# spirit-man/Planetary-LiDAR-Odometry

Hardware: AMD Instinct MI355X
Metric: IMLS-ICP scan-pairs/s (HDL-64 ~120k-pt scan vs 10-scan map, 20 ICP iterations) (higher is better)
Workload: dtype f64; 1 GPU; config B: HDL-64 scan vs 10-scan local map; a step = 4 independent scan pairs as 4 launch sequences in flight; queries=126189, map_points=1262664, solver=LS (trimmed, t=0.02), search_number=20, inputs=resident in HBM, fused_launch=True, launch_groups=4, parallelism=1 GPU, no process group

## Files before the change

planetary-lidar-odometry_amd/csrc/internal.h:

```cpp
#pragma once
#include <cstddef>
#include <hip/hip_runtime.h>
#include <cstdint>
#include <string>
#include <vector>

#include "../../include/imls_gpu.h"

namespace imlsgpu {

constexpr int kBlock = 256;
constexpr int kProjBlock = 128;
constexpr int kStackDepth = 24;
constexpr int kHistBins = 65536;
constexpr int kCandCap = 8192;
constexpr int kNormEq = 28;

static_assert(sizeof(imls_iter_trace) == 16 * 8 * 2 + 8 * 8, "trace layout");

struct DevBuf {
    void* p = nullptr;
    size_t bytes = 0;
};

// ... 16 lines not shown
    double delta_dist, delta_angle;
    int matcher;
    int proj;
    double gate_dist, gate_proj;
    int qwave;
    int packet;
    int pk_small, pk_iters;
    int pk_batch;
    int reuse;
    int force_fb;
    int xcd;
    int tv;
    int tv_k;
    double tv_sigma, tv_thr;
    float tv_skin;
    int bfs;
};
#ifndef IMLS_BFS_ITERS
#define IMLS_BFS_ITERS 0
#endif
inline KParams kp_at(const KParams& k, int it) {
    KParams r = k;
    r.packet = it >= 0 && it < k.pk_iters ? k.pk_small : 64;
    r.bfs = it >= 0 && it < IMLS_BFS_ITERS;
    return r;
}
constexpr int kTvMaxK = 64;
constexpr int kTvList = 64;
constexpr size_t kTvBytesPerQuery = 32 + 16 + 4 * kTvList + 72;

struct TreeView {
    const float4* mpt;
    const float4* mnr;
    const unsigned* ipos;
    const float4* nodes;
    const float4* tpt;
    const float4* tnr;
    int M, B, P, levels;
    const unsigned long long* lkeys;
// ... 211 lines not shown
int fifo_merge(hipStream_t s, const unsigned long long* a, const unsigned* av, int na, const unsigned long long* b,
               unsigned bid, int nb, unsigned long long* okey, unsigned* oval, DevBuf& scratch, std::string& err);
int fifo_index(hipStream_t s, const unsigned long long* mkey, const unsigned* mval, int M, const FifoRunTable& runs,
               const float* fq, const unsigned* clamp, unsigned* h_clamp, int B, DevBuf& lkeys, DevBuf& mpt, DevBuf& nodes,
               DevBuf& treescratch, int* P_out, int* levels_out, std::string& err);

void launch_project(hipStream_t s, const TreeView& t, const float4* spt, const float4* snr,
                    const unsigned* qperm, int N, const double* pose, const int* done, const KParams& kp,
                    float4* cs, float4* cd, float4* cn, double* partial1, imls_iter_trace* tr,
                    unsigned long long* nbr_stats, unsigned* fb_list, unsigned* fb_count, int lane_mode,
                    const double* delta, int* lists, int use_prev, hipEvent_t* marks = nullptr);
constexpr int kMaxKL = 46;
__host__ __device__ inline float4* xref_of(int* lists, int N) {
    return reinterpret_cast<float4*>(reinterpret_cast<char*>(lists) + ((size_t)(kMaxKL + 1) * N * 4 + 255) / 256 * 256);
}
__host__ __device__ inline unsigned* cmp_of(int* lists, int N) {
    return reinterpret_cast<unsigned*>(reinterpret_cast<char*>(xref_of(lists, N)) + ((size_t)N * 20 + 255) / 256 * 256);
}
__host__ __device__ inline unsigned* cmp_count_of(int* lists, int N) { return cmp_of(lists, N) + ((size_t)N + 63) / 64 * 64; }
inline size_t prevnn_bytes(int N) {
    return ((size_t)(kMaxKL + 1) * N * 4 + 255) / 256 * 256 + ((size_t)N * 20 + 255) / 256 * 256 + ((size_t)N + 63) / 64 * 256 +
           ((size_t)N / 64 + 2) * 4 + 512;
}
constexpr int kStatSkipped = 6;
int project_blocks(int N);
#ifndef IMLS_FINISH_QUAD
#define IMLS_FINISH_QUAD 0
#endif
constexpr int kPass1Block = IMLS_FINISH_QUAD ? 64 : 256;
constexpr int kPass1Fallback = 64;
void launch_project_batch(hipStream_t s, const PairDev* tab, const int* n_host, int npairs, const KParams& kp, int it,
                          int use_prev);

void launch_solve_chain(hipStream_t s, int N, int blocks1, const KParams& kp, const float4* cs,
                        const float4* cd, const float4* cn, const double* rows_d, const double* weights,
                        SolveState& st, imls_iter_trace* tr, int update_pose, int rows_are_double,
                        const int* count = nullptr, const double* wsum = nullptr);
// ... 63 lines not shown
```

planetary-lidar-odometry_amd/csrc/project.hip:

```cpp
#include <algorithm>
#include <cfloat>

#include "internal.h"
#include "geom.h"

namespace imlsgpu {
namespace {

constexpr double kInfD = __builtin_huge_val();
constexpr float kInfF = __builtin_huge_valf();
constexpr int kWaveBlock = 256;
typedef float kf4v __attribute__((ext_vector_type(4)));
typedef __attribute__((address_space(4))) const kf4v kconst_f4;
__device__ __forceinline__ int ld_const(const int* p) { return *(const __attribute__((address_space(4))) int*)p; }
__device__ __forceinline__ double ld_const(const double* p) { return *(const __attribute__((address_space(4))) double*)p; }
constexpr int kFallbackBlocks = 64;
constexpr int kFallbackBlocksBatched = 4;
constexpr int kFinishPerBlock = IMLS_FINISH_QUAD ? kWaveBlock / 4 : kWaveBlock;
static_assert(kFinishPerBlock == kPass1Block && kFallbackBlocks == kPass1Fallback, "pass-1 slab layout (solve.hip)");
#ifndef IMLS_COMPACT
#define IMLS_COMPACT 0
#endif
constexpr int kWideMax = 8;
constexpr int kWaveStack = 64;
constexpr int kFStack = 256;
constexpr int kFBatchMax = 128;
static_assert(kFBatchMax + 64 + 7 * ((24 + 2) / 3) <= kFStack, "frontier stack bound");
#ifndef IMLS_SEED_CHUNK
#define IMLS_SEED_CHUNK 8
#endif
constexpr int kSeedChunk = IMLS_SEED_CHUNK;
constexpr int kSeedTab = 1024;
constexpr int kSeedHalf = 1;
constexpr float kReseed = 0.25f;
#ifndef IMLS_LEAF_PREFETCH
#define IMLS_LEAF_PREFETCH 1
#endif
// ... 336 lines not shown
#pragma unroll
    for (int j = 0; j < KL; ++j) {
        const float up = I::hi(lk[j]);
        const bool in = I::real(lk[j]) && up <= r2f;
        cnt_r += in ? 1 : 0;
        if (in && d1 == kInfF && I::lo(lk[j]) > 1e-15f) d1 = up;
        if (j == K - 1) dK = up;
    }
    return cnt_r >= K ? fmaxf(dK, d1) : (IMLS_UNDER_SKIN > 0 ? r2f : kInfF);
}

#ifndef IMLS_KNN_WAVES
#define IMLS_KNN_WAVES 5
#endif
#define IMLS_KNN_ATTR __attribute__((amdgpu_waves_per_eu(KL <= 26 ? IMLS_KNN_WAVES : 2)))
template <int KL, int MODE = 0>
__device__ __forceinline__ void knn_wave_body(TreeView t, const float4* __restrict__ spt,
                                                         const unsigned* __restrict__ qperm, int N,
                                                         const double* __restrict__ pose,
                                                         const int* __restrict__ done, KParams kp,
                                                         const double* __restrict__ delta,
                                                         int* __restrict__ lists, float* __restrict__ wlist,
                                                         float4* __restrict__ xref, float* __restrict__ nref,
                                                         int use_prev, unsigned long long* __restrict__ nbr_stats,
                                                         int bx, unsigned* __restrict__ cmp = nullptr,
                                                         unsigned* __restrict__ cmp_count = nullptr) {
    if (done && ld_const(done)) return;
    __shared__ int snode[kWaveBlock / 64][kWaveStack];
    __shared__ float4 sboxa[kWaveBlock / 64][kWaveStack];
    __shared__ float2 sboxb[kWaveBlock / 64][kWaveStack];
    __shared__ int spos[KL][kWaveBlock];
    const int tid = threadIdx.x, lane = tid & 63;
    int* const mypos = &spos[0][tid];
    using IK = IdKeys<KL>;
    const int wv = __builtin_amdgcn_readfirstlane(tid >> 6);
    const int qp = kp.packet;
    const int pslot = (bx * (kWaveBlock / 64) + wv) * qp + lane;
    int slot = pslot;
    bool active = lane < qp && slot < N;
    if constexpr (MODE == 2) {
        const int cnt = ld_const((const int*)cmp_count + bx);
        if (wv * qp >= cnt) return;
        active = lane < qp && wv * qp + lane < cnt;
        slot = active ? (int)cmp[(size_t)bx * (kWaveBlock / 64) * qp + wv * qp + lane] : 0;
    }
    float xf[3] = {0.f, 0.f, 0.f};
    float w_prev = 0.f, n_prev = 0.f;
    float4 x_prev = make_float4(0.f, 0.f, 0.f, 0.f);
    if (active) {
        double ns[3];
        const int i = (int)qperm[slot];
        const float4 sp4 = spt[i];
        if (use_prev) {
            w_prev = wlist[slot];
            x_prev = xref[slot];
            n_prev = nref[slot];
        }
        transform_query(pose, sp4, make_float4(0.f, 0.f, 0.f, 0.f), 0, xf, ns);
    }
    float lk[KL];
// ... 2 lines not shown
    if (use_prev) {
#pragma unroll
        for (int j = 0; j < KL; ++j) mypos[j * kWaveBlock] = -1;
    }
    auto thr_ = [&]() -> float { return IK::lo(lk[KL - 1]); };
    auto full_ = [&]() -> bool { return IK::real(lk[KL - 1]); };
    auto pos_ = [&](int s) -> int { return mypos[s * kWaveBlock]; };
    auto need_ = [&]() -> float { return need_key_ids<KL>(lk, (float)kp.r2, kp.K); };
    auto ins_ = [&](float d, int pos) {
        const unsigned s = IK::id(lk[KL - 1]);
        insert_key<KL>(lk, IK::make(d, s));
        mypos[s * kWaveBlock] = pos;
    };
    const float r2s = (float)(kp.r2 * kSearchR2) * kBoxSlack + 1e-30f;
    float bnd = active ? r2s : -1.0f;
    const int P = t.P, B = t.B, M = t.M;
#ifdef IMLS_DEBUG_WAVE_TRACE
    const long long dbg_t0 = wall_clock64();
#endif
    bool greedy = active && !use_prev;
    bool skip = false;
    float wskip = kInfF;
    if (active && use_prev) {
        double rf = 0.0;
#pragma unroll
        for (int r = 0; r < 3; ++r)
#pragma unroll
            for (int c = 0; c < 3; ++c) {
                const double e = ld_const(delta + r * 4 + c) - (r == c ? 1.0 : 0.0);
                rf += e * e;
            }
// ... 38 lines not shown
                for (int j = par; j + 1 < KL; j += 2) {
                    const bool sw = lk[j + 1] < lk[j];
                    const float tk = lk[j];
                    lk[j] = sw ? lk[j + 1] : lk[j];
                    lk[j + 1] = sw ? tk : lk[j + 1];
                    swapped |= sw;
                }
            }
        }
        bnd = fmin_nn(r2s, thr_());
        if (kp.reuse && wlow > 0.f) {
            const float nk = need_();
            if (nk < kInfF && nk * (1.0f + 1e-5f) < wlow) { skip = true; wskip = wlow; }
        }
    }
    if constexpr (MODE == 1) {
        if (active && skip) wlist[slot] = wskip;
        const unsigned long long sk = __ballot(skip);
        if (nbr_stats && lane == 0 && sk) atomicAdd(&nbr_stats[kStatSkipped], (unsigned long long)__popcll(sk));
        const bool need = active && !skip;
        const unsigned long long nm = __ballot(need);
        __shared__ int wneed[kWaveBlock / 64];
        if (lane == 0) wneed[wv] = __popcll(nm);
        __syncthreads();
        int off = 0, tot = 0;
#pragma unroll
        for (int w = 0; w < kWaveBlock / 64; ++w) {
            off += w < wv ? wneed[w] : 0;
            tot += wneed[w];
        }
        if (need) cmp[(size_t)bx * (kWaveBlock / 64) * qp + off + __popcll(nm & ((1ull << lane) - 1ull))] = (unsigned)slot;
        if (tid == 0) cmp_count[bx] = (unsigned)tot;
        return;
    }
#ifdef IMLS_DEBUG_WAVE_TRACE
    unsigned dbg_ev = 0, dbg_ins = 0;
    unsigned dbg_sparse = 0, dbg_bcast = 0, dbg_sparse_lanes = 0, dbg_sparse_ins = 0;
    unsigned dbg_seed_steps = 0, dbg_seed_pts = 0;
#endif
    auto scan_leaf = [&](int leaf, unsigned long long want, bool listed, float4 mine) {
        const int base = leaf * B;
        const int cnt = min(B, M - base);
        unsigned long long inl = 0ull;
        auto listed_mask = [&]() {
#pragma unroll
            for (int k = 0; k < KL; ++k) {
                const unsigned rel = (unsigned)(pos_(k) - base);
                inl |= rel < 64u ? (1ull << rel) : 0ull;
            }
        };
        const bool sparse = __popcll(want) <= kSparseLanes;
#ifdef IMLS_DEBUG_WAVE_TRACE
        if (sparse) { ++dbg_sparse; dbg_sparse_lanes += __popcll(want); } else { ++dbg_bcast; }
#endif
        if (sparse) {
            int nin = 0;
            bool have_inl = !listed;
            if (listed) {
#pragma unroll
                for (int k = 0; k < KL; ++k) nin += (unsigned)(pos_(k) - base) < (unsigned)cnt ? 1 : 0;
            }
            const float cb = fmin_nn(r2s, IK::hi(lk[KL - 1]));
            unsigned long long cm = 0ull;
            unsigned long long m = want;
            while (m) {
                const int q = __builtin_amdgcn_readfirstlane(__builtin_ctzll(m));
                m &= m - 1;
                const float qx = __int_as_float(__builtin_amdgcn_readlane(__float_as_int(xf[0]), q));
                const float qy = __int_as_float(__builtin_amdgcn_readlane(__float_as_int(xf[1]), q));
                const float qz = __int_as_float(__builtin_amdgcn_readlane(__float_as_int(xf[2]), q));
                const float qb = __int_as_float(__builtin_amdgcn_readlane(__float_as_int(cb), q));
                const float ex = mine.x - qx, ey = mine.y - qy, ez = mine.z - qz;
                const float d32 = __builtin_fmaf(ex, ex, __builtin_fmaf(ey, ey, ez * ez));
                unsigned long long pm = __ballot(lane < cnt && d32 <= qb);
                if (!have_inl) {
                    const int nq = __builtin_amdgcn_readlane(nin, q);
                    if (__popcll(pm) > nq) {
                        listed_mask();
                        have_inl = true;
                    } else {
                        pm = 0ull;
                    }
                }
                if (pm) {
                    const unsigned long long inq =
                        ((unsigned long long)(unsigned)__builtin_amdgcn_readlane((int)(unsigned)(inl >> 32), q) << 32) |
                        (unsigned)__builtin_amdgcn_readlane((int)(unsigned)inl, q);
                    pm &= ~inq;
                }
                if (lane == q) cm = pm;
            }
            while (__ballot(cm != 0ull)) {
                const int jj = cm ? (int)__builtin_ctzll(cm) : 0;
                const float px = __shfl(mine.x, jj), py = __shfl(mine.y, jj), pz = __shfl(mine.z, jj);
                if (cm) {
                    cm &= cm - 1;
                    const float ex = px - xf[0], ey = py - xf[1], ez = pz - xf[2];
                    const float d32 = __builtin_fmaf(ex, ex, __builtin_fmaf(ey, ey, ez * ez));
                    if (d32 <= bnd && d32 < thr_()) {
#ifdef IMLS_DEBUG_WAVE_TRACE
                        ++dbg_ins;
#endif
                        ins_(d32, base + jj);
                        bnd = fmin_nn(r2s, thr_());
                    }
                }
#ifdef IMLS_DEBUG_WAVE_TRACE
                ++dbg_ev;
#endif
            }
        } else {
            if (listed) listed_mask();
            const bool wants = (want >> lane) & 1ull;
#if IMLS_BCAST_SCALAR
            const kconst_f4* lp = (const kconst_f4*)t.mpt + base;
            kf4v g[kBcGroup];
#pragma unroll
            for (int u = 0; u < kBcGroup; ++u) g[u] = lp[min(u, cnt - 1)];
            for (int j0 = 0; j0 < cnt; j0 += kBcGroup) {
                kf4v nx[kBcGroup];
                const int jn = j0 + kBcGroup;
                if (jn + kBcGroup <= cnt) {
                    const kconst_f4* q = lp + jn;
#pragma unroll
                    for (int u = 0; u < kBcGroup; ++u) nx[u] = q[u];
                } else {
// ... 103 lines not shown
        }
    }
    unsigned n_inner = 0, n_leaf = 0;
#ifdef IMLS_DEBUG_WAVE_TRACE
    const long long dbg_t1 = wall_clock64();
#endif
    if (skip) bnd = -1.0f;
    int node = 1, sp = 0;
#if IMLS_LEAF_PREFETCH
    int pf_leaf = -1;
    float4 pf = make_float4(0.f, 0.f, 0.f, 0.f);
#endif
    unsigned long long em = __ballot(active && !skip);
    const unsigned long long skipped = __ballot(skip);
    if (nbr_stats && lane == 0 && skipped) atomicAdd(&nbr_stats[kStatSkipped], (unsigned long long)__popcll(skipped));
    if constexpr (MODE == 3) {
        if (em) {
            const bool walk = active && !skip;
            const float rr = walk ? sqrtf(bnd * kBoxSlack) * (1.0f + 1e-5f) + 1e-5f : 0.f;
            float plo[3], phi[3];
#pragma unroll
            for (int a = 0; a < 3; ++a) {
                plo[a] = walk ? xf[a] - rr : kInfF;
                phi[a] = walk ? xf[a] + rr : -kInfF;
            }
#pragma unroll
            for (int o = 1; o < 64; o <<= 1)
#pragma unroll
                for (int a = 0; a < 3; ++a) {
                    plo[a] = fminf(plo[a], __shfl_xor(plo[a], o, 64));
                    phi[a] = fmaxf(phi[a], __shfl_xor(phi[a], o, 64));
                }
            int fc = 1, lev = 0;
            if (lane == 0) snode[wv][0] = 1;
            while (lev < t.levels) {
                const int sw = min(kWide, t.levels - lev), nk = 1 << sw;
                const int below = t.levels - lev - sw;
                const int reserve = (kWideMax - 1) * ((below + kWide - 1) / kWide);
                const int n = lane < fc ? snode[wv][lane] : 0;
                const float4* rec = t.nodes + 3 * ((size_t)(n > 0 ? n : 1) << (sw - 1));
                auto child_box = [&](int k, float (&lo)[3], float (&hi)[3]) {
                    const float4 ra = rec[3 * (k >> 1)], rb = rec[3 * (k >> 1) + 1], rc = rec[3 * (k >> 1) + 2];
                    if (k & 1) { lo[0] = rb.z; lo[1] = rb.w; lo[2] = rc.x; hi[0] = rc.y; hi[1] = rc.z; hi[2] = rc.w; }
                    else { lo[0] = ra.x; lo[1] = ra.y; lo[2] = ra.z; hi[0] = ra.w; hi[1] = rb.x; hi[2] = rb.y; }
                };
                unsigned cm = 0u;
                if (lane < fc) {
#pragma unroll
                    for (int k = 0; k < kWideMax; ++k) {
                        if (k >= nk) break;
                        float lo[3], hi[3];
                        child_box(k, lo, hi);
                        const bool ov = lo[0] <= phi[0] && hi[0] >= plo[0] && lo[1] <= phi[1] && hi[1] >= plo[1] &&
                                        lo[2] <= phi[2] && hi[2] >= plo[2];
                        cm |= ov ? (1u << k) : 0u;
                    }
                }
                const int cnt = __popc(cm);
                int inc = cnt;
#pragma unroll
                for (int o = 1; o < 64; o <<= 1) {
                    const int v = __shfl_up(inc, o, 64);
                    if (lane >= o) inc += v;
                }
                const int total = __shfl(inc, 63, 64);
                if (total == 0 || total + reserve > kWaveStack) break;
                int off = inc - cnt;
                if (cm) {
#pragma unroll
                    for (int k = 0; k < kWideMax; ++k) {
                        if (!((cm >> k) & 1u)) continue;
                        float lo[3], hi[3];
                        child_box(k, lo, hi);
                        snode[wv][off] = (n << sw) + k;
                        sboxa[wv][off] = make_float4(lo[0], lo[1], lo[2], hi[0]);
                        sboxb[wv][off] = make_float2(hi[1], hi[2]);
                        ++off;
                    }
                }
                fc = total;
                lev += sw;
                ++n_inner;
            }
            if (lev > 0) {
                int en = 0;
                float4 ea = make_float4(0.f, 0.f, 0.f, 0.f);
                float2 eb = make_float2(0.f, 0.f);
                if (lane < fc) { en = snode[wv][lane]; ea = sboxa[wv][lane]; eb = sboxb[wv][lane]; }
                if (lane < fc) { snode[wv][fc - 1 - lane] = en; sboxa[wv][fc - 1 - lane] = ea; sboxb[wv][fc - 1 - lane] = eb; }
                sp = fc;
                node = 0;
                while (sp > 0) {
                    --sp;
                    const float4 b0 = sboxa[wv][sp];
                    const float2 b1 = sboxb[wv][sp];
                    const float d = box_d2(xf, b0.x, b0.y, b0.z, b0.w, b1.x, b1.y);
                    em = __ballot(d <= bnd * kBoxSlack);
                    if (em) { node = snode[wv][sp]; break; }
                }
                if (!node) em = 0ull;
            }
        }
    }
    while (em) {
        if (node < P) {
            ++n_inner;
            const int lev = 31 - __builtin_clz(node);
            const int sw = min(kWide, t.levels - lev);
            const int nk = 1 << sw, nrec = nk >> 1;
            const int unode = __builtin_amdgcn_readfirstlane(node);
            const kconst_f4* rec = (const kconst_f4*)t.nodes + 3 * ((size_t)unode << (sw - 1));
            float4 R[3 * (kWideMax / 2)];
#pragma unroll
            for (int k = 0; k < 3 * (kWideMax / 2); ++k) {
                const kf4v v = rec[min(k, 3 * nrec - 1)];
                R[k] = make_float4(v.x, v.y, v.z, v.w);
            }
            const float bs = bnd * kBoxSlack;
            unsigned long long m[kWideMax];
            int best = -1;
            float bd = kInfF;
#pragma unroll
            for (int k = 0; k < kWideMax; ++k) {
                const float4 a = R[3 * (k >> 1)], b = R[3 * (k >> 1) + 1], c = R[3 * (k >> 1) + 2];
                const float d = (k & 1) ? box_d2(xf, b.z, b.w, c.x, c.y, c.z, c.w) : box_d2(xf, a.x, a.y, a.z, a.w, b.x, b.y);
                const bool w = k < nk && d <= bs;
                m[k] = __ballot(w);
                if (w && d < bd) { bd = d; best = k; }
            }
            int cstar = -1, vbest = 0;
#pragma unroll
            for (int k = 0; k < kWideMax; ++k) {
                const int v = __popcll(__ballot(best == k));
                if (m[k] && (cstar < 0 || v > vbest)) { cstar = k; vbest = v; }
            }
            if (cstar >= 0) {
#pragma unroll
                for (int k = kWideMax - 1; k >= 0; --k) {
                    if (m[k] && k != cstar) {
                        if (lane == 0) {
                            const float4 a = R[3 * (k >> 1)], b = R[3 * (k >> 1) + 1], c = R[3 * (k >> 1) + 2];
                            snode[wv][sp] = (node << sw) + k;
                            sboxa[wv][sp] = (k & 1) ? make_float4(b.z, b.w, c.x, c.y) : make_float4(a.x, a.y, a.z, a.w);
                            sboxb[wv][sp] = (k & 1) ? make_float2(c.z, c.w) : make_float2(b.x, b.y);
                        }
                        ++sp;
                    }
                }
                em = m[cstar];
                node = (node << sw) + cstar;
                continue;
            }
        } else {
            ++n_leaf;
            const int leaf = node - P;
            float4 mine = make_float4(0.f, 0.f, 0.f, 0.f);
#if IMLS_LEAF_PREFETCH
            if (leaf == pf_leaf) mine = pf;
            else if (lane < min(B, M - leaf * B)) mine = t.mpt[leaf * B + lane];
            pf_leaf = -1;
            if (sp > 0) {
                const int nn = __builtin_amdgcn_readfirstlane(snode[wv][sp - 1]);
                if (nn >= P) {
                    pf_leaf = nn - P;
                    pf = make_float4(0.f, 0.f, 0.f, 0.f);
                    if (lane < min(B, M - pf_leaf * B)) pf = t.mpt[pf_leaf * B + lane];
                }
            }
#else
            if ((!IMLS_BCAST_SCALAR || __popcll(em) <= kSparseLanes) && lane < min(B, M - leaf * B))
                mine = t.mpt[leaf * B + lane];
#endif
            scan_leaf(leaf, em, use_prev || gmask, mine);
        }
        node = 0;
        while (sp > 0) {
            --sp;
            const float4 b0 = sboxa[wv][sp];
            const float2 b1 = sboxb[wv][sp];
            const float d = box_d2(xf, b0.x, b0.y, b0.z, b0.w, b1.x, b1.y);
            em = __ballot(d <= bnd * kBoxSlack);
            if (em) { node = snode[wv][sp]; break; }
        }
        if (!node) break;
    }
    if (active && skip) wlist[slot] = wskip;
    if (active && !skip) {
#pragma unroll
        for (int j = 0; j < KL; ++j) lists[(size_t)j * N + slot] = pos_(IK::id(lk[j]));
        const bool full = full_();
        const float wk = full ? thr_() : kInfF;
        wlist[slot] = wk;
        xref[slot] = make_float4(xf[0], xf[1], xf[2], full ? wk : r2s);
        nref[slot] = need_();
    }
#ifdef IMLS_DEBUG_WAVE_TRACE
    if (nbr_stats && lane == 0) {
        atomicAdd(&nbr_stats[6], (unsigned long long)dbg_ev);
        atomicAdd(&nbr_stats[7], (unsigned long long)dbg_ins);
// ... 2 lines not shown
        const long long dbg_t2 = wall_clock64();
        atomicAdd(&nbr_stats[8], (unsigned long long)(dbg_t1 - dbg_t0));
        atomicMax(&nbr_stats[9], (unsigned long long)(dbg_t1 - dbg_t0));
        atomicAdd(&nbr_stats[10], (unsigned long long)(dbg_t2 - dbg_t1));
        atomicMax(&nbr_stats[11], (unsigned long long)(dbg_t2 - dbg_t1));
        atomicAdd(&nbr_stats[12], (unsigned long long)n_leaf);
        atomicMax(&nbr_stats[13], (unsigned long long)n_leaf);
        atomicMax(&nbr_stats[14], (unsigned long long)dbg_ev);
        atomicAdd(&nbr_stats[15], (unsigned long long)__popcll(__ballot(greedy)));
    }
    {
        const unsigned long long gl = __ballot(greedy), wi = __ballot(active && !full_()),
                                 w1 = __ballot(active && full_() && thr_() > 1.0f);
        float wmax = active && full_() ? thr_() : 0.f;
        for (int o = 1; o < 64; o <<= 1) wmax = fmaxf(wmax, __shfl_xor(wmax, o));
        unsigned sins = dbg_sparse_ins;
        for (int o = 1; o < 64; o <<= 1) sins += __shfl_xor(sins, o);
        if (lane == 0) {
            const int w = bx * (kWaveBlock / 64) + wv;
            if (w < kDbgWaves) {
                unsigned* r = g_dbg_wave[w];
                r[0] = (unsigned)(dbg_t1 - dbg_t0); r[1] = (unsigned)(wall_clock64() - dbg_t1);
                r[2] = n_leaf; r[3] = n_inner; r[4] = dbg_ev; r[5] = dbg_sparse; r[6] = dbg_bcast;
                r[7] = __popcll(gl); r[8] = __popcll(wi); r[9] = __popcll(w1); r[10] = __float_as_uint(wmax);
                r[11] = dbg_sparse_lanes; r[12] = sins; r[13] = dbg_ins;
                r[14] = dbg_seed_steps; r[15] = __builtin_amdgcn_readfirstlane(dbg_seed_pts);
            }
        }
    }
#endif
    if (nbr_stats && lane == 0) {
        atomicAdd(&nbr_stats[2], (unsigned long long)n_leaf);
        atomicAdd(&nbr_stats[3], (unsigned long long)n_inner);
        atomicAdd(&nbr_stats[4], 1ull);
    }
}

template <int KL>
__device__ __forceinline__ void finish_q_core(TreeView t, const float4* __restrict__ spt, const float4* __restrict__ snr,
                                              int i, int slot, const double* __restrict__ pose, const KParams& kp,
// ... 1210 lines not shown
    if (nbr_stats && tid >= IMLS_NUM_REJ && tid < IMLS_NUM_REJ + 2 && rej_s[tid])
        atomicAdd(&nbr_stats[tid - IMLS_NUM_REJ], (unsigned long long)rej_s[tid]);
}

template <int KL>
__global__ __launch_bounds__(kWaveBlock) IMLS_KNN_ATTR void k_knn_wave(
        TreeView t, const float4* __restrict__ spt, const unsigned* __restrict__ qperm, int N,
        const double* __restrict__ pose, const int* __restrict__ done, KParams kp, const double* __restrict__ delta,
        int* __restrict__ lists, float* __restrict__ wlist, float4* __restrict__ xref, float* __restrict__ nref,
        int use_prev, unsigned long long* __restrict__ nbr_stats) {
    knn_wave_body<KL>(t, spt, qperm, N, pose, done, kp, delta, lists, wlist, xref, nref, use_prev, nbr_stats,
                      (int)blockIdx.x);
}

template <int KL>
__global__ __launch_bounds__(kWaveBlock) IMLS_KNN_ATTR void k_knn_wave_bfs(
        TreeView t, const float4* __restrict__ spt, const unsigned* __restrict__ qperm, int N,
        const double* __restrict__ pose, const int* __restrict__ done, KParams kp, const double* __restrict__ delta,
        int* __restrict__ lists, float* __restrict__ wlist, float4* __restrict__ xref, float* __restrict__ nref,
        int use_prev, unsigned long long* __restrict__ nbr_stats) {
    knn_wave_body<KL, 3>(t, spt, qperm, N, pose, done, kp, delta, lists, wlist, xref, nref, use_prev, nbr_stats,
                         (int)blockIdx.x);
}

template <int KL, int MODE>
__global__ __launch_bounds__(kWaveBlock) IMLS_KNN_ATTR void k_knn_wave_m(
        TreeView t, const float4* __restrict__ spt, const unsigned* __restrict__ qperm, int N,
        const double* __restrict__ pose, const int* __restrict__ done, KParams kp, const double* __restrict__ delta,
        int* __restrict__ lists, float* __restrict__ wlist, float4* __restrict__ xref, float* __restrict__ nref,
        unsigned long long* __restrict__ nbr_stats) {
    knn_wave_body<KL, MODE>(t, spt, qperm, N, pose, done, kp, delta, lists, wlist, xref, nref, 1, nbr_stats,
                            (int)blockIdx.x, cmp_of(lists, N), cmp_count_of(lists, N));
}

template <int KL>
__global__ __launch_bounds__(kWaveBlock) void k_knn_qwave(
        TreeView t, const float4* __restrict__ spt, const unsigned* __restrict__ qperm, int N,
        const double* __restrict__ pose, const int* __restrict__ done, KParams kp, const double* __restrict__ delta,
        int* __restrict__ lists, float* __restrict__ wlist, float4* __restrict__ xref, float* __restrict__ nref,
        int use_prev, unsigned long long* __restrict__ nbr_stats) {
    knn_qwave_body<KL>(t, spt, qperm, N, pose, done, kp, delta, lists, wlist, xref, nref, use_prev, nbr_stats,
                       (int)blockIdx.x);
}

template <int KL>
__global__ __launch_bounds__(kWaveBlock) void k_knn_qwave_f(
        TreeView t, const float4* __restrict__ spt, const unsigned* __restrict__ qperm, int N,
        const double* __restrict__ pose, const int* __restrict__ done, KParams kp, const double* __restrict__ delta,
        int* __restrict__ lists, float* __restrict__ wlist, float4* __restrict__ xref, float* __restrict__ nref,
        int use_prev, unsigned long long* __restrict__ nbr_stats, QFinishArgs fa) {
// ... 59 lines not shown
    bx = (int)(s % nx);
}

template <int KL>
__global__ __launch_bounds__(kWaveBlock) IMLS_KNN_ATTR void k_knn_wave_b(const PairDev* __restrict__ tab, KParams kp,
                                                                          int use_prev, int npairs) {
    int f, bx;
    batch_block(kp.xcd, f, bx);
    if (f >= npairs) return;
    const PairDev A = device_view(tab + f);
    if (use_qwave(kp, A.N) || bx >= knn_blocks_of(A.N, kp.packet)) return;
    float4* xref = xref_dev(A.lists, A.N);
    knn_wave_body<KL>(A.t, A.spt, A.qperm, A.N, A.st.pose, A.st.done, kp, A.st.delta, A.lists,
                                wlist_of<KL>(A.lists, A.N), xref, reinterpret_cast<float*>(xref + A.N), use_prev, A.stats,
                                bx);
}

template <int KL>
__global__ __launch_bounds__(kWaveBlock) IMLS_KNN_ATTR void k_knn_wave_bfsb(const PairDev* __restrict__ tab, KParams kp,
                                                                             int use_prev, int npairs) {
    int f, bx;
    batch_block(kp.xcd, f, bx);
    if (f >= npairs) return;
    const PairDev A = device_view(tab + f);
    if (use_qwave(kp, A.N) || bx >= knn_blocks_of(A.N, kp.packet)) return;
    float4* xref = xref_dev(A.lists, A.N);
    knn_wave_body<KL, 3>(A.t, A.spt, A.qperm, A.N, A.st.pose, A.st.done, kp, A.st.delta, A.lists,
                         wlist_of<KL>(A.lists, A.N), xref, reinterpret_cast<float*>(xref + A.N), use_prev, A.stats, bx);
}

template <int KL, int MODE>
__global__ __launch_bounds__(kWaveBlock) IMLS_KNN_ATTR void k_knn_wave_mb(const PairDev* __restrict__ tab, KParams kp,
                                                                           int npairs) {
    int f, bx;
    batch_block(kp.xcd, f, bx);
    if (f >= npairs) return;
    const PairDev A = device_view(tab + f);
    if (use_qwave(kp, A.N) || bx >= knn_blocks_of(A.N, kp.packet)) return;
    float4* xref = xref_dev(A.lists, A.N);
    knn_wave_body<KL, MODE>(A.t, A.spt, A.qperm, A.N, A.st.pose, A.st.done, kp, A.st.delta, A.lists,
                            wlist_of<KL>(A.lists, A.N), xref, reinterpret_cast<float*>(xref + A.N), 1, A.stats, bx,
                            cmp_of(A.lists, A.N), cmp_count_of(A.lists, A.N));
}

template <int KL>
__global__ __launch_bounds__(kWaveBlock) void k_knn_qwave_b(const PairDev* __restrict__ tab, KParams kp, int use_prev,
                                                            int npairs) {
    int f, bx;
    batch_block(kp.xcd, f, bx);
    if (f >= npairs) return;
    const PairDev A = device_view(tab + f);
    if (!use_qwave(kp, A.N) || bx * (kWaveBlock / 64) >= A.N) return;
    float4* xref = xref_dev(A.lists, A.N);
    knn_qwave_body<KL>(A.t, A.spt, A.qperm, A.N, A.st.pose, A.st.done, kp, A.st.delta, A.lists, wlist_of<KL>(A.lists, A.N),
                       xref, reinterpret_cast<float*>(xref + A.N), use_prev, A.stats, bx);
}

// ... 21 lines not shown
                            A.st.partial1 + (size_t)finish_blocks_of(A.N) * kNormEq, A.trace + it, A.stats,
                            kFallbackBlocks);
}

template <int KL>
void launch_wave_batch(hipStream_t s, const PairDev* tab, int npairs, int maxN, bool any_small, bool any_large,
                       const KParams& kp, int it, int use_prev) {
    const int wb = finish_blocks_of(maxN);
    const int gy = kp.xcd ? (npairs + 7) / 8 * 8 : npairs;
    if (any_small) {
        const int n = kp.qwave > 0 ? maxN : std::min(maxN, kQwaveAutoN);
        k_knn_qwave_b<KL><<<dim3((n + kWaveBlock / 64 - 1) / (kWaveBlock / 64), gy), kWaveBlock, 0, s>>>(tab, kp, use_prev, npairs);
    }
    if (any_large) {
        const int kb = knn_blocks_of(maxN, kp.packet);
        if (it < IMLS_BFS_ITERS) {
            k_knn_wave_bfsb<KL><<<dim3(kb, gy), kWaveBlock, 0, s>>>(tab, kp, use_prev, npairs);
        } else if (use_prev && IMLS_COMPACT) {
            k_knn_wave_mb<KL, 1><<<dim3(kb, gy), kWaveBlock, 0, s>>>(tab, kp, npairs);
            k_knn_wave_mb<KL, 2><<<dim3(kb, gy), kWaveBlock, 0, s>>>(tab, kp, npairs);
        } else {
            k_knn_wave_b<KL><<<dim3(kb, gy), kWaveBlock, 0, s>>>(tab, kp, use_prev, npairs);
        }
    }
    k_finish_b<KL><<<dim3(wb, gy), kWaveBlock, 0, s>>>(tab, kp, it, npairs);
}

template <int KCAP>
void launch_lane(hipStream_t s, int blocks, const TreeView& t, const float4* spt, const float4* snr, const unsigned* qlist,
                 const unsigned* qcount, int N, const double* pose, const int* done, const KParams& kp, float4* cs,
                 float4* cd, float4* cn, double* partial1, imls_iter_trace* tr, unsigned long long* stats) {
    k_project_lane<KCAP><<<blocks, kProjBlock, 0, s>>>(t, spt, snr, qlist, qcount, N, pose, done, kp, cs, cd, cn, partial1,
                                                       tr, stats);
}


#ifndef IMLS_LONE_EXTRA
#define IMLS_LONE_EXTRA 10
// ... 6 lines not shown
                 int N, const double* pose, const int* done, const KParams& kp, float4* cs, float4* cd, float4* cn,
                 double* partial1, imls_iter_trace* tr, unsigned long long* stats, unsigned* fb_list, unsigned* fb_count,
                 const double* delta, int* lists, int use_prev, hipEvent_t* marks) {
    float* wlist = reinterpret_cast<float*>(lists + (size_t)KL * N);
    float4* xref = xref_of(lists, N);
    float* nref = reinterpret_cast<float*>(xref + N);
    if (marks) (void)hipEventRecord(marks[0], s);
    const bool fused = fused_stage(kp, N);
    if (fused)
        k_knn_qwave_f<lone_kl<KL>()><<<(N + kWaveBlock / 64 - 1) / (kWaveBlock / 64), kWaveBlock, 0, s>>>(
            t, spt, qperm, N, pose, done, kp, delta, lists, reinterpret_cast<float*>(lists + (size_t)lone_kl<KL>() * N), xref,
            nref, use_prev, stats, QFinishArgs{snr, cs, cd, cn, tr});
    else if (use_qwave(kp, N))
        k_knn_qwave<KL><<<(N + kWaveBlock / 64 - 1) / (kWaveBlock / 64), kWaveBlock, 0, s>>>(t, spt, qperm, N, pose, done, kp,
                                                                                          delta, lists, wlist, xref, nref, use_prev, stats);
    else if (kp.bfs && IMLS_BFS_ITERS > 0)
        k_knn_wave_bfs<KL><<<knn_blocks_of(N, kp.packet), kWaveBlock, 0, s>>>(t, spt, qperm, N, pose, done, kp, delta, lists,
                                                                              wlist, xref, nref, use_prev, stats);
    else if (use_prev && IMLS_COMPACT) {
        k_knn_wave_m<KL, 1><<<knn_blocks_of(N, kp.packet), kWaveBlock, 0, s>>>(t, spt, qperm, N, pose, done, kp, delta, lists,
                                                                               wlist, xref, nref, stats);
        k_knn_wave_m<KL, 2><<<knn_blocks_of(N, kp.packet), kWaveBlock, 0, s>>>(t, spt, qperm, N, pose, done, kp, delta, lists,
                                                                               wlist, xref, nref, stats);
    } else
        k_knn_wave<KL><<<knn_blocks_of(N, kp.packet), kWaveBlock, 0, s>>>(t, spt, qperm, N, pose, done, kp, delta, lists, wlist,
                                                                          xref, nref, use_prev, stats);
    if (marks) (void)hipEventRecord(marks[1], s);
    if (!fused)
        k_finish<KL><<<blocks, kWaveBlock, 0, s>>>(t, spt, snr, qperm, N, pose, done, kp, lists, wlist, cs, cd, cn, partial1,
                                                   tr, stats, fb_list, fb_count);
    if (marks) (void)hipEventRecord(marks[2], s);
}

}

void launch_project_batch(hipStream_t s, const PairDev* tab, const int* n_host, int npairs, const KParams& kp0, int it,
                          int use_prev) {
    KParams kp = kp_at(kp0, kp0.pk_batch ? it : -1);
    long long total = 0;
// ... 61 lines not shown
```

Before: 447.9 scan-pairs/s.

## Make wave kNN traversal control flow uniform and drop unused BFS/compact modes

Removes the disabled BFS-frontier and compaction kNN modes along with their kernels and buffer space. In the active wave kNN body it forces the tree sizes, leaf-vs-inner and pop decisions into scalar registers, and builds the per-lane candidate masks with writelane instead of a lane compare. Child-box stack pushes now run in parallel across lanes from per-lane loads instead of a serial lane-0 loop. The sparse and broadcast leaf paths become separate scalar-gated blocks. The aim is less divergence and fewer serialized steps in the traversal loop, at the cost of extra per-lane child-box loads and some asm register pinning that may hurt the compiler's scheduling.

```diff
diff --git a/planetary-lidar-odometry_amd/csrc/internal.h b/planetary-lidar-odometry_amd/csrc/internal.h
--- a/planetary-lidar-odometry_amd/csrc/internal.h
+++ b/planetary-lidar-odometry_amd/csrc/internal.h
@@ -54,15 +54,10 @@
     int tv_k;
     double tv_sigma, tv_thr;
     float tv_skin;
-    int bfs;
-};
-#ifndef IMLS_BFS_ITERS
-#define IMLS_BFS_ITERS 0
-#endif
+};
 inline KParams kp_at(const KParams& k, int it) {
     KParams r = k;
     r.packet = it >= 0 && it < k.pk_iters ? k.pk_small : 64;
-    r.bfs = it >= 0 && it < IMLS_BFS_ITERS;
     return r;
 }
 constexpr int kTvMaxK = 64;
@@ -304,13 +299,8 @@
 __host__ __device__ inline float4* xref_of(int* lists, int N) {
     return reinterpret_cast<float4*>(reinterpret_cast<char*>(lists) + ((size_t)(kMaxKL + 1) * N * 4 + 255) / 256 * 256);
 }
-__host__ __device__ inline unsigned* cmp_of(int* lists, int N) {
-    return reinterpret_cast<unsigned*>(reinterpret_cast<char*>(xref_of(lists, N)) + ((size_t)N * 20 + 255) / 256 * 256);
-}
-__host__ __device__ inline unsigned* cmp_count_of(int* lists, int N) { return cmp_of(lists, N) + ((size_t)N + 63) / 64 * 64; }
 inline size_t prevnn_bytes(int N) {
-    return ((size_t)(kMaxKL + 1) * N * 4 + 255) / 256 * 256 + ((size_t)N * 20 + 255) / 256 * 256 + ((size_t)N + 63) / 64 * 256 +
-           ((size_t)N / 64 + 2) * 4 + 512;
+    return ((size_t)(kMaxKL + 1) * N * 4 + 255) / 256 * 256 + ((size_t)N * 20 + 255) / 256 * 256 + 512;
 }
 constexpr int kStatSkipped = 6;
 int project_blocks(int N);
diff --git a/planetary-lidar-odometry_amd/csrc/project.hip b/planetary-lidar-odometry_amd/csrc/project.hip
--- a/planetary-lidar-odometry_amd/csrc/project.hip
+++ b/planetary-lidar-odometry_amd/csrc/project.hip
@@ -3,6 +3,14 @@
 
 #include "internal.h"
 #include "geom.h"
+
+#if defined(__has_builtin) && __has_builtin(__builtin_amdgcn_writelane)
+__device__ __forceinline__ int imls_amdgcn_writelane(int v, int sel, int old) {
+    return __builtin_amdgcn_writelane(v, sel, old);
+}
+#else
+__device__ int imls_amdgcn_writelane(int v, int sel, int old) __asm("llvm.amdgcn.writelane");
+#endif
 
 namespace imlsgpu {
 namespace {
@@ -18,9 +26,6 @@
 constexpr int kFallbackBlocksBatched = 4;
 constexpr int kFinishPerBlock = IMLS_FINISH_QUAD ? kWaveBlock / 4 : kWaveBlock;
 static_assert(kFinishPerBlock == kPass1Block && kFallbackBlocks == kPass1Fallback, "pass-1 slab layout (solve.hip)");
-#ifndef IMLS_COMPACT
-#define IMLS_COMPACT 0
-#endif
 constexpr int kWideMax = 8;
 constexpr int kWaveStack = 64;
 constexpr int kFStack = 256;
@@ -387,7 +392,7 @@
 #define IMLS_KNN_WAVES 5
 #endif
 #define IMLS_KNN_ATTR __attribute__((amdgpu_waves_per_eu(KL <= 26 ? IMLS_KNN_WAVES : 2)))
-template <int KL, int MODE = 0>
+template <int KL>
 __device__ __forceinline__ void knn_wave_body(TreeView t, const float4* __restrict__ spt,
                                                          const unsigned* __restrict__ qperm, int N,
                                                          const double* __restrict__ pose,
@@ -396,8 +401,7 @@
                                                          int* __restrict__ lists, float* __restrict__ wlist,
                                                          float4* __restrict__ xref, float* __restrict__ nref,
                                                          int use_prev, unsigned long long* __restrict__ nbr_stats,
-                                                         int bx, unsigned* __restrict__ cmp = nullptr,
-                                                         unsigned* __restrict__ cmp_count = nullptr) {
+                                                         int bx) {
     if (done && ld_const(done)) return;
     __shared__ int snode[kWaveBlock / 64][kWaveStack];
     __shared__ float4 sboxa[kWaveBlock / 64][kWaveStack];
@@ -408,15 +412,8 @@
     using IK = IdKeys<KL>;
     const int wv = __builtin_amdgcn_readfirstlane(tid >> 6);
     const int qp = kp.packet;
-    const int pslot = (bx * (kWaveBlock / 64) + wv) * qp + lane;
-    int slot = pslot;
-    bool active = lane < qp && slot < N;
-    if constexpr (MODE == 2) {
-        const int cnt = ld_const((const int*)cmp_count + bx);
-        if (wv * qp >= cnt) return;
-        active = lane < qp && wv * qp + lane < cnt;
-        slot = active ? (int)cmp[(size_t)bx * (kWaveBlock / 64) * qp + wv * qp + lane] : 0;
-    }
+    const int slot = (bx * (kWaveBlock / 64) + wv) * qp + lane;
+    const bool active = lane < qp && slot < N;
     float xf[3] = {0.f, 0.f, 0.f};
     float w_prev = 0.f, n_prev = 0.f;
     float4 x_prev = make_float4(0.f, 0.f, 0.f, 0.f);
@@ -449,7 +446,8 @@
     };
     const float r2s = (float)(kp.r2 * kSearchR2) * kBoxSlack + 1e-30f;
     float bnd = active ? r2s : -1.0f;
-    const int P = t.P, B = t.B, M = t.M;
+    int P = t.P, B = t.B, M = t.M;
+    asm volatile("" : "+s"(P), "+s"(B), "+s"(M));
 #ifdef IMLS_DEBUG_WAVE_TRACE
     const long long dbg_t0 = wall_clock64();
 #endif
@@ -518,28 +516,9 @@
             if (nk < kInfF && nk * (1.0f + 1e-5f) < wlow) { skip = true; wskip = wlow; }
         }
     }
-    if constexpr (MODE == 1) {
-        if (active && skip) wlist[slot] = wskip;
-        const unsigned long long sk = __ballot(skip);
-        if (nbr_stats && lane == 0 && sk) atomicAdd(&nbr_stats[kStatSkipped], (unsigned long long)__popcll(sk));
-        const bool need = active && !skip;
-        const unsigned long long nm = __ballot(need);
-        __shared__ int wneed[kWaveBlock / 64];
-        if (lane == 0) wneed[wv] = __popcll(nm);
-        __syncthreads();
-        int off = 0, tot = 0;
-#pragma unroll
-        for (int w = 0; w < kWaveBlock / 64; ++w) {
-            off += w < wv ? wneed[w] : 0;
-            tot += wneed[w];
-        }
-        if (need) cmp[(size_t)bx * (kWaveBlock / 64) * qp + off + __popcll(nm & ((1ull << lane) - 1ull))] = (unsigned)slot;
-        if (tid == 0) cmp_count[bx] = (unsigned)tot;
-        return;
-    }
 #ifdef IMLS_DEBUG_WAVE_TRACE
     unsigned dbg_ev = 0, dbg_ins = 0;
-    unsigned dbg_sparse = 0, dbg_bcast = 0, dbg_sparse_lanes = 0, dbg_sparse_ins = 0;
+    unsigned dbg_sparse = 0, dbg_bcast = 0, dbg_sparse_lanes = 0, dbg_listed_lv = 0;
     unsigned dbg_seed_steps = 0, dbg_seed_pts = 0;
 #endif
     auto scan_leaf = [&](int leaf, unsigned long long want, bool listed, float4 mine) {
@@ -554,6 +533,8 @@
             }
         };
         const bool sparse = __popcll(want) <= kSparseLanes;
+        int bcast = __builtin_amdgcn_readfirstlane(!sparse);
+        asm volatile("" : "+s"(bcast));
 #ifdef IMLS_DEBUG_WAVE_TRACE
         if (sparse) { ++dbg_sparse; dbg_sparse_lanes += __popcll(want); } else { ++dbg_bcast; }
 #endif
@@ -563,9 +544,13 @@
             if (listed) {
 #pragma unroll
                 for (int k = 0; k < KL; ++k) nin += (unsigned)(pos_(k) - base) < (unsigned)cnt ? 1 : 0;
+#ifdef IMLS_DEBUG_WAVE_TRACE
+                dbg_listed_lv += (__ballot(nin > 0) & want) ? 1 : 0;
+#endif
             }
             const float cb = fmin_nn(r2s, IK::hi(lk[KL - 1]));
-            unsigned long long cm = 0ull;
+            int cm_lo = 0, cm_hi = 0;
+            const unsigned long long inleaf = cnt >= 64 ? ~0ull : (1ull << max(cnt, 0)) - 1ull;
             unsigned long long m = want;
             while (m) {
                 const int q = __builtin_amdgcn_readfirstlane(__builtin_ctzll(m));
@@ -576,7 +561,7 @@
                 const float qb = __int_as_float(__builtin_amdgcn_readlane(__float_as_int(cb), q));
                 const float ex = mine.x - qx, ey = mine.y - qy, ez = mine.z - qz;
                 const float d32 = __builtin_fmaf(ex, ex, __builtin_fmaf(ey, ey, ez * ez));
-                unsigned long long pm = __ballot(lane < cnt && d32 <= qb);
+                unsigned long long pm = __ballot(d32 <= qb) & inleaf;
                 if (!have_inl) {
                     const int nq = __builtin_amdgcn_readlane(nin, q);
                     if (__popcll(pm) > nq) {
@@ -592,8 +577,10 @@
                         (unsigned)__builtin_amdgcn_readlane((int)(unsigned)inl, q);
                     pm &= ~inq;
                 }
-                if (lane == q) cm = pm;
-            }
+                cm_lo = imls_amdgcn_writelane((int)(unsigned)pm, q, cm_lo);
+                cm_hi = imls_amdgcn_writelane((int)(unsigned)(pm >> 32), q, cm_hi);
+            }
+            unsigned long long cm = ((unsigned long long)(unsigned)cm_hi << 32) | (unsigned)cm_lo;
             while (__ballot(cm != 0ull)) {
                 const int jj = cm ? (int)__builtin_ctzll(cm) : 0;
                 const float px = __shfl(mine.x, jj), py = __shfl(mine.y, jj), pz = __shfl(mine.z, jj);
@@ -613,7 +600,8 @@
                 ++dbg_ev;
 #endif
             }
-        } else {
+        }
+        if (bcast) {
             if (listed) listed_mask();
             const bool wants = (want >> lane) & 1ull;
 #if IMLS_BCAST_SCALAR
@@ -747,95 +735,10 @@
     unsigned long long em = __ballot(active && !skip);
     const unsigned long long skipped = __ballot(skip);
     if (nbr_stats && lane == 0 && skipped) atomicAdd(&nbr_stats[kStatSkipped], (unsigned long long)__popcll(skipped));
-    if constexpr (MODE == 3) {
-        if (em) {
-            const bool walk = active && !skip;
-            const float rr = walk ? sqrtf(bnd * kBoxSlack) * (1.0f + 1e-5f) + 1e-5f : 0.f;
-            float plo[3], phi[3];
-#pragma unroll
-            for (int a = 0; a < 3; ++a) {
-                plo[a] = walk ? xf[a] - rr : kInfF;
-                phi[a] = walk ? xf[a] + rr : -kInfF;
-            }
-#pragma unroll
-            for (int o = 1; o < 64; o <<= 1)
-#pragma unroll
-                for (int a = 0; a < 3; ++a) {
-                    plo[a] = fminf(plo[a], __shfl_xor(plo[a], o, 64));
-                    phi[a] = fmaxf(phi[a], __shfl_xor(phi[a], o, 64));
-                }
-            int fc = 1, lev = 0;
-            if (lane == 0) snode[wv][0] = 1;
-            while (lev < t.levels) {
-                const int sw = min(kWide, t.levels - lev), nk = 1 << sw;
-                const int below = t.levels - lev - sw;
-                const int reserve = (kWideMax - 1) * ((below + kWide - 1) / kWide);
-                const int n = lane < fc ? snode[wv][lane] : 0;
-                const float4* rec = t.nodes + 3 * ((size_t)(n > 0 ? n : 1) << (sw - 1));
-                auto child_box = [&](int k, float (&lo)[3], float (&hi)[3]) {
-                    const float4 ra = rec[3 * (k >> 1)], rb = rec[3 * (k >> 1) + 1], rc = rec[3 * (k >> 1) + 2];
-                    if (k & 1) { lo[0] = rb.z; lo[1] = rb.w; lo[2] = rc.x; hi[0] = rc.y; hi[1] = rc.z; hi[2] = rc.w; }
-                    else { lo[0] = ra.x; lo[1] = ra.y; lo[2] = ra.z; hi[0] = ra.w; hi[1] = rb.x; hi[2] = rb.y; }
-                };
-                unsigned cm = 0u;
-                if (lane < fc) {
-#pragma unroll
-                    for (int k = 0; k < kWideMax; ++k) {
-                        if (k >= nk) break;
-                        float lo[3], hi[3];
-                        child_box(k, lo, hi);
-                        const bool ov = lo[0] <= phi[0] && hi[0] >= plo[0] && lo[1] <= phi[1] && hi[1] >= plo[1] &&
-                                        lo[2] <= phi[2] && hi[2] >= plo[2];
-                        cm |= ov ? (1u << k) : 0u;
-                    }
-                }
-                const int cnt = __popc(cm);
-                int inc = cnt;
-#pragma unroll
-                for (int o = 1; o < 64; o <<= 1) {
-                    const int v = __shfl_up(inc, o, 64);
-                    if (lane >= o) inc += v;
-                }
-                const int total = __shfl(inc, 63, 64);
-                if (total == 0 || total + reserve > kWaveStack) break;
-                int off = inc - cnt;
-                if (cm) {
-#pragma unroll
-                    for (int k = 0; k < kWideMax; ++k) {
-                        if (!((cm >> k) & 1u)) continue;
-                        float lo[3], hi[3];
-                        child_box(k, lo, hi);
-                        snode[wv][off] = (n << sw) + k;
-                        sboxa[wv][off] = make_float4(lo[0], lo[1], lo[2], hi[0]);
-                        sboxb[wv][off] = make_float2(hi[1], hi[2]);
-                        ++off;
-                    }
-                }
-                fc = total;
-                lev += sw;
-                ++n_inner;
-            }
-            if (lev > 0) {
-                int en = 0;
-                float4 ea = make_float4(0.f, 0.f, 0.f, 0.f);
-                float2 eb = make_float2(0.f, 0.f);
-                if (lane < fc) { en = snode[wv][lane]; ea = sboxa[wv][lane]; eb = sboxb[wv][lane]; }
-                if (lane < fc) { snode[wv][fc - 1 - lane] = en; sboxa[wv][fc - 1 - lane] = ea; sboxb[wv][fc - 1 - lane] = eb; }
-                sp = fc;
-                node = 0;
-                while (sp > 0) {
-                    --sp;
-                    const float4 b0 = sboxa[wv][sp];
-                    const float2 b1 = sboxb[wv][sp];
-                    const float d = box_d2(xf, b0.x, b0.y, b0.z, b0.w, b1.x, b1.y);
-                    em = __ballot(d <= bnd * kBoxSlack);
-                    if (em) { node = snode[wv][sp]; break; }
-                }
-                if (!node) em = 0ull;
-            }
-        }
-    }
     while (em) {
+        int pop = 1;
+        int at_leaf = __builtin_amdgcn_readfirstlane(node >= P);
+        asm volatile("" : "+s"(at_leaf));
         if (node < P) {
             ++n_inner;
             const int lev = 31 - __builtin_clz(node);
@@ -843,6 +746,11 @@
             const int nk = 1 << sw, nrec = nk >> 1;
             const int unode = __builtin_amdgcn_readfirstlane(node);
             const kconst_f4* rec = (const kconst_f4*)t.nodes + 3 * ((size_t)unode << (sw - 1));
+            float2 cb0 = make_float2(0.f, 0.f), cb1 = cb0, cb2 = cb0;
+            if (lane < nk) {
+                const float2* cp = reinterpret_cast<const float2*>(t.nodes + 3 * ((size_t)unode << (sw - 1))) + 3 * lane;
+                cb0 = cp[0]; cb1 = cp[1]; cb2 = cp[2];
+            }
             float4 R[3 * (kWideMax / 2)];
 #pragma unroll
             for (int k = 0; k < 3 * (kWideMax / 2); ++k) {
@@ -862,29 +770,30 @@
                 if (w && d < bd) { bd = d; best = k; }
             }
             int cstar = -1, vbest = 0;
+            unsigned long long mstar = 0ull;
 #pragma unroll
             for (int k = 0; k < kWideMax; ++k) {
                 const int v = __popcll(__ballot(best == k));
-                if (m[k] && (cstar < 0 || v > vbest)) { cstar = k; vbest = v; }
+                if (m[k] && (cstar < 0 || v > vbest)) { cstar = k; vbest = v; mstar = m[k]; }
+            }
+            unsigned wm = 0u;
+#pragma unroll
+            for (int k = 0; k < kWideMax; ++k) wm |= m[k] ? (1u << k) : 0u;
+            const unsigned pm = cstar >= 0 ? wm & ~(1u << cstar) : 0u;
+            if (lane < kWideMax && ((pm >> lane) & 1u)) {
+                const int pos = sp + __popc(pm >> (lane + 1));
+                snode[wv][pos] = (node << sw) + lane;
+                sboxa[wv][pos] = make_float4(cb0.x, cb0.y, cb1.x, cb1.y);
+                sboxb[wv][pos] = cb2;
             }
             if (cstar >= 0) {
-#pragma unroll
-                for (int k = kWideMax - 1; k >= 0; --k) {
-                    if (m[k] && k != cstar) {
-                        if (lane == 0) {
-                            const float4 a = R[3 * (k >> 1)], b = R[3 * (k >> 1) + 1], c = R[3 * (k >> 1) + 2];
-                            snode[wv][sp] = (node << sw) + k;
-                            sboxa[wv][sp] = (k & 1) ? make_float4(b.z, b.w, c.x, c.y) : make_float4(a.x, a.y, a.z, a.w);
-                            sboxb[wv][sp] = (k & 1) ? make_float2(c.z, c.w) : make_float2(b.x, b.y);
-                        }
-                        ++sp;
-                    }
-                }
-                em = m[cstar];
+                sp += __popc(pm);
+                em = mstar;
                 node = (node << sw) + cstar;
-                continue;
-            }
-        } else {
+                pop = 0;
+            }
+        }
+        if (at_leaf) {
             ++n_leaf;
             const int leaf = node - P;
             float4 mine = make_float4(0.f, 0.f, 0.f, 0.f);
@@ -906,16 +815,18 @@
 #endif
             scan_leaf(leaf, em, use_prev || gmask, mine);
         }
-        node = 0;
-        while (sp > 0) {
-            --sp;
-            const float4 b0 = sboxa[wv][sp];
-            const float2 b1 = sboxb[wv][sp];
-            const float d = box_d2(xf, b0.x, b0.y, b0.z, b0.w, b1.x, b1.y);
-            em = __ballot(d <= bnd * kBoxSlack);
-            if (em) { node = snode[wv][sp]; break; }
-        }
-        if (!node) break;
+        asm volatile("" : "+s"(pop));
+        if (pop) {
+            em = 0ull;
+            while (sp > 0 && !em) {
+                --sp;
+                const float4 b0 = sboxa[wv][sp];
+                const float2 b1 = sboxb[wv][sp];
+                const float d = box_d2(xf, b0.x, b0.y, b0.z, b0.w, b1.x, b1.y);
+                em = __ballot(d <= bnd * kBoxSlack);
+            }
+            if (em) node = snode[wv][sp];
+        }
     }
     if (active && skip) wlist[slot] = wskip;
     if (active && !skip) {
@@ -948,8 +859,6 @@
                                  w1 = __ballot(active && full_() && thr_() > 1.0f);
         float wmax = active && full_() ? thr_() : 0.f;
         for (int o = 1; o < 64; o <<= 1) wmax = fmaxf(wmax, __shfl_xor(wmax, o));
-        unsigned sins = dbg_sparse_ins;
-        for (int o = 1; o < 64; o <<= 1) sins += __shfl_xor(sins, o);
         if (lane == 0) {
             const int w = bx * (kWaveBlock / 64) + wv;
             if (w < kDbgWaves) {
@@ -957,7 +866,7 @@
                 r[0] = (unsigned)(dbg_t1 - dbg_t0); r[1] = (unsigned)(wall_clock64() - dbg_t1);
                 r[2] = n_leaf; r[3] = n_inner; r[4] = dbg_ev; r[5] = dbg_sparse; r[6] = dbg_bcast;
                 r[7] = __popcll(gl); r[8] = __popcll(wi); r[9] = __popcll(w1); r[10] = __float_as_uint(wmax);
-                r[11] = dbg_sparse_lanes; r[12] = sins; r[13] = dbg_ins;
+                r[11] = dbg_sparse_lanes; r[12] = dbg_listed_lv; r[13] = dbg_ins;
                 r[14] = dbg_seed_steps; r[15] = __builtin_amdgcn_readfirstlane(dbg_seed_pts);
             }
         }
@@ -2198,26 +2107,6 @@
 }
 
 template <int KL>
-__global__ __launch_bounds__(kWaveBlock) IMLS_KNN_ATTR void k_knn_wave_bfs(
-        TreeView t, const float4* __restrict__ spt, const unsigned* __restrict__ qperm, int N,
-        const double* __restrict__ pose, const int* __restrict__ done, KParams kp, const double* __restrict__ delta,
-        int* __restrict__ lists, float* __restrict__ wlist, float4* __restrict__ xref, float* __restrict__ nref,
-        int use_prev, unsigned long long* __restrict__ nbr_stats) {
-    knn_wave_body<KL, 3>(t, spt, qperm, N, pose, done, kp, delta, lists, wlist, xref, nref, use_prev, nbr_stats,
-                         (int)blockIdx.x);
-}
-
-template <int KL, int MODE>
-__global__ __launch_bounds__(kWaveBlock) IMLS_KNN_ATTR void k_knn_wave_m(
-        TreeView t, const float4* __restrict__ spt, const unsigned* __restrict__ qperm, int N,
-        const double* __restrict__ pose, const int* __restrict__ done, KParams kp, const double* __restrict__ delta,
-        int* __restrict__ lists, float* __restrict__ wlist, float4* __restrict__ xref, float* __restrict__ nref,
-        unsigned long long* __restrict__ nbr_stats) {
-    knn_wave_body<KL, MODE>(t, spt, qperm, N, pose, done, kp, delta, lists, wlist, xref, nref, 1, nbr_stats,
-                            (int)blockIdx.x, cmp_of(lists, N), cmp_count_of(lists, N));
-}
-
-template <int KL>
 __global__ __launch_bounds__(kWaveBlock) void k_knn_qwave(
         TreeView t, const float4* __restrict__ spt, const unsigned* __restrict__ qperm, int N,
         const double* __restrict__ pose, const int* __restrict__ done, KParams kp, const double* __restrict__ delta,
@@ -2307,33 +2196,6 @@
     knn_wave_body<KL>(A.t, A.spt, A.qperm, A.N, A.st.pose, A.st.done, kp, A.st.delta, A.lists,
                                 wlist_of<KL>(A.lists, A.N), xref, reinterpret_cast<float*>(xref + A.N), use_prev, A.stats,
                                 bx);
-}
-
-template <int KL>
-__global__ __launch_bounds__(kWaveBlock) IMLS_KNN_ATTR void k_knn_wave_bfsb(const PairDev* __restrict__ tab, KParams kp,
-                                                                             int use_prev, int npairs) {
-    int f, bx;
-    batch_block(kp.xcd, f, bx);
-    if (f >= npairs) return;
-    const PairDev A = device_view(tab + f);
-    if (use_qwave(kp, A.N) || bx >= knn_blocks_of(A.N, kp.packet)) return;
-    float4* xref = xref_dev(A.lists, A.N);
-    knn_wave_body<KL, 3>(A.t, A.spt, A.qperm, A.N, A.st.pose, A.st.done, kp, A.st.delta, A.lists,
-                         wlist_of<KL>(A.lists, A.N), xref, reinterpret_cast<float*>(xref + A.N), use_prev, A.stats, bx);
-}
-
-template <int KL, int MODE>
-__global__ __launch_bounds__(kWaveBlock) IMLS_KNN_ATTR void k_knn_wave_mb(const PairDev* __restrict__ tab, KParams kp,
-                                                                           int npairs) {
-    int f, bx;
-    batch_block(kp.xcd, f, bx);
-    if (f >= npairs) return;
-    const PairDev A = device_view(tab + f);
-    if (use_qwave(kp, A.N) || bx >= knn_blocks_of(A.N, kp.packet)) return;
-    float4* xref = xref_dev(A.lists, A.N);
-    knn_wave_body<KL, MODE>(A.t, A.spt, A.qperm, A.N, A.st.pose, A.st.done, kp, A.st.delta, A.lists,
-                            wlist_of<KL>(A.lists, A.N), xref, reinterpret_cast<float*>(xref + A.N), 1, A.stats, bx,
-                            cmp_of(A.lists, A.N), cmp_count_of(A.lists, A.N));
 }
 
 template <int KL>
@@ -2385,14 +2247,7 @@
     }
     if (any_large) {
         const int kb = knn_blocks_of(maxN, kp.packet);
-        if (it < IMLS_BFS_ITERS) {
-            k_knn_wave_bfsb<KL><<<dim3(kb, gy), kWaveBlock, 0, s>>>(tab, kp, use_prev, npairs);
-        } else if (use_prev && IMLS_COMPACT) {
-            k_knn_wave_mb<KL, 1><<<dim3(kb, gy), kWaveBlock, 0, s>>>(tab, kp, npairs);
-            k_knn_wave_mb<KL, 2><<<dim3(kb, gy), kWaveBlock, 0, s>>>(tab, kp, npairs);
-        } else {
-            k_knn_wave_b<KL><<<dim3(kb, gy), kWaveBlock, 0, s>>>(tab, kp, use_prev, npairs);
-        }
+        k_knn_wave_b<KL><<<dim3(kb, gy), kWaveBlock, 0, s>>>(tab, kp, use_prev, npairs);
     }
     k_finish_b<KL><<<dim3(wb, gy), kWaveBlock, 0, s>>>(tab, kp, it, npairs);
 }
@@ -2429,15 +2284,7 @@
     else if (use_qwave(kp, N))
         k_knn_qwave<KL><<<(N + kWaveBlock / 64 - 1) / (kWaveBlock / 64), kWaveBlock, 0, s>>>(t, spt, qperm, N, pose, done, kp,
                                                                                           delta, lists, wlist, xref, nref, use_prev, stats);
-    else if (kp.bfs && IMLS_BFS_ITERS > 0)
-        k_knn_wave_bfs<KL><<<knn_blocks_of(N, kp.packet), kWaveBlock, 0, s>>>(t, spt, qperm, N, pose, done, kp, delta, lists,
-                                                                              wlist, xref, nref, use_prev, stats);
-    else if (use_prev && IMLS_COMPACT) {
-        k_knn_wave_m<KL, 1><<<knn_blocks_of(N, kp.packet), kWaveBlock, 0, s>>>(t, spt, qperm, N, pose, done, kp, delta, lists,
-                                                                               wlist, xref, nref, stats);
-        k_knn_wave_m<KL, 2><<<knn_blocks_of(N, kp.packet), kWaveBlock, 0, s>>>(t, spt, qperm, N, pose, done, kp, delta, lists,
-                                                                               wlist, xref, nref, stats);
-    } else
+    else
         k_knn_wave<KL><<<knn_blocks_of(N, kp.packet), kWaveBlock, 0, s>>>(t, spt, qperm, N, pose, done, kp, delta, lists, wlist,
                                                                           xref, nref, use_prev, stats);
     if (marks) (void)hipEventRecord(marks[1], s);
```

Result: faster. 469.9 scan-pairs/s, median of 6 (+4.9%).
